# SajayR/TRIAD

Measured on AMD Instinct MI355X. Metric: tri-modal triples/sec (whole node) + loss parity, B=256 at 1/2/4/8 MI355X, higher is better.
Workload: dtype bf16

## Files before the change

triad_amd/csrc/attention.hip:

```cpp
#include "attention_tiles.h"

namespace {

constexpr int MAX_KT = 10;

struct AttnArgs {
  const bf16 *q, *k, *v, *o, *dout;
  long long q_sB, q_sN, k_sB, k_sN, v_sB, v_sN, o_sB, o_sN, do_sB, do_sN;
  bf16 *out, *dq, *dk, *dv;
  long long out_sB, out_sN, dq_sB, dq_sN, dk_sB, dk_sN, dv_sB, dv_sN;
  float* lse;
  float* delta;
  int B, H, N;
  float scale;
  const unsigned *wq, *wk;
  int nkt;
  float drop_scale;
};

template <int NT>
__device__ __forceinline__ void load_rows2(char* l0, const bf16* b0, long long s0, char* l1, const bf16* b1,
                                           long long s1, int N) {
  static_assert((NT * 32 * 8) % 256 == 0, "256 threads");
  constexpr int PER = NT * 32 * 8 / 256;
  bf16x8 r0[PER], r1[PER];
#pragma unroll
  for (int i = 0; i < PER; ++i) {
    const int e = threadIdx.x + 256 * i, r = e >> 3, c = e & 7;
    r0[i] = r < N ? *(const bf16x8*)(b0 + (long long)r * s0 + c * 8) : (bf16x8){};
    r1[i] = r < N ? *(const bf16x8*)(b1 + (long long)r * s1 + c * 8) : (bf16x8){};
  }
#pragma unroll
  for (int i = 0; i < PER; ++i) {
    const int e = threadIdx.x + 256 * i, r = e >> 3, c = e & 7;
    const int off = r * 128 + ((c ^ swz(r)) << 4);
    *(bf16x8*)(l0 + off) = r0[i];
    *(bf16x8*)(l1 + off) = r1[i];
  }
}

template <int NKT, bool DROP>
__global__ __launch_bounds__(256, 2) void attn_fwd_kernel(AttnArgs a) {
  __shared__ __attribute__((aligned(16))) char lds[2 * NKT * 32 * 128];
  char* kl = lds;
  char* vl = lds + NKT * 32 * 128;
  const int bh = blockIdx.y, b = bh / a.H, hh = bh - b * a.H;
  const int lane = threadIdx.x & 63, wave = threadIdx.x >> 6, h = lane >> 5, ql = lane & 31;
  const int qt = blockIdx.x * 4 + wave;
  const int q = qt * 32 + ql;
  const bool qok = q < a.N;
  bf16x8 qf[4];
  {
    const bf16* qp = a.q + b * a.q_sB + (long long)(qok ? q : 0) * a.q_sN + hh * HD + 8 * h;
#pragma unroll
    for (int s = 0; s < 4; ++s) qf[s] = qok ? *(const bf16x8*)(qp + 16 * s) : (bf16x8){};
  }
  load_rows2<NKT>(kl, a.k + b * a.k_sB + hh * HD, a.k_sN, vl, a.v + b * a.v_sB + hh * HD, a.v_sN, a.N);
  __syncthreads();
  if (qt * 32 >= a.N) return;
  f32x16 acc[NKT];
#pragma unroll
  for (int kt = 0; kt < NKT; ++kt) {
    acc[kt] = (f32x16){};
#pragma unroll
    for (int s = 0; s < 4; ++s) acc[kt] = mfma32(lds_b128(kl, kt * 32 + ql, 2 * s + h), qf[s], acc[kt]);
  }
  const int nlast = a.N - (NKT - 1) * 32;
  if (nlast < 32) {
#pragma unroll
    for (int v = 0; v < 16; ++v)
      if ((v & 3) + 8 * (v >> 2) + 4 * h >= nlast) acc[NKT - 1][v] = -INFINITY;
  }
  float m = -INFINITY;
#pragma unroll
  for (int kt = 0; kt < NKT; ++kt)
#pragma unroll
    for (int v = 0; v < 16; ++v) m = fmaxf(m, acc[kt][v]);
  m = fmaxf(m, __shfl_xor(m, 32));
  const float c2 = a.scale * LOG2E;
  const float mo = m * c2;
  float l = 0.f;
#pragma unroll
  for (int kt = 0; kt < NKT; ++kt)
#pragma unroll
    for (int v = 0; v < 16; ++v) {
      const float p = __builtin_amdgcn_exp2f(fmaf(acc[kt][v], c2, -mo));
      acc[kt][v] = p;
      l += p;
    }
  l += __shfl_xor(l, 32);
  if (DROP) {
#pragma unroll
    for (int kt = 0; kt < NKT; ++kt) {
      const unsigned w = qok ? a.wq[((long long)bh * a.N + q) * NKT + kt] : 0u;
#pragma unroll
      for (int v = 0; v < 16; ++v) acc[kt][v] = tile_bit(w, v, h) ? acc[kt][v] : 0.f;
    }
  }

  f32x16 o0 = {}, o1 = {};
#pragma unroll
  for (int kt = 0; kt < NKT; ++kt)
#pragma unroll
    for (int half = 0; half < 2; ++half) {
      const int c = 2 * kt + half;
      const bf16x8 pf = pack8(acc[kt], half);
      o0 = mfma32(frag_tr(vl, c, 0, lane), pf, o0);
      o1 = mfma32(frag_tr(vl, c, 32, lane), pf, o1);
    }
  if (!qok) return;
  const float inv = (DROP ? a.drop_scale : 1.f) / l;
  bf16* op = a.out + b * a.out_sB + (long long)q * a.out_sN + hh * HD;
  store_cols(op, o0, inv, h);
  store_cols(op + 32, o1, inv, h);
  if (h == 0) a.lse[(long long)bh * a.N + q] = m * a.scale + logf(l);
}

template <int NKT, bool DROP>
__global__ __launch_bounds__(256, 2) void attn_dq_kernel(AttnArgs a) {
  __shared__ __attribute__((aligned(16))) char lds[2 * NKT * 32 * 128];
  char* kl = lds;
  char* vl = lds + NKT * 32 * 128;
  const int bh = blockIdx.y, b = bh / a.H, hh = bh - b * a.H;
  const int lane = threadIdx.x & 63, wave = threadIdx.x >> 6, h = lane >> 5, ql = lane & 31;
  const int qt = blockIdx.x * 4 + wave;
  const int q = qt * 32 + ql;
  const bool qok = q < a.N;
  bf16x8 qf[4], df[4], ov[4];
  {
    const long long qq = qok ? q : 0;
    const bf16* qp = a.q + b * a.q_sB + qq * a.q_sN + hh * HD + 8 * h;
    const bf16* dp = a.dout + b * a.do_sB + qq * a.do_sN + hh * HD + 8 * h;
    const bf16* op = a.o + b * a.o_sB + qq * a.o_sN + hh * HD + 8 * h;
#pragma unroll
    for (int s = 0; s < 4; ++s) {
      qf[s] = qok ? *(const bf16x8*)(qp + 16 * s) : (bf16x8){};
      df[s] = qok ? *(const bf16x8*)(dp + 16 * s) : (bf16x8){};
      ov[s] = qok ? *(const bf16x8*)(op + 16 * s) : (bf16x8){};
    }
  }
  const float lse2 = qok ? a.lse[(long long)bh * a.N + q] * LOG2E : 0.f;
  load_rows2<NKT>(kl, a.k + b * a.k_sB + hh * HD, a.k_sN, vl, a.v + b * a.v_sB + hh * HD, a.v_sN, a.N);
  __syncthreads();
  if (qt * 32 >= a.N) return;
  float dl = 0.f;
#pragma unroll
  for (int s = 0; s < 4; ++s)
#pragma unroll
    for (int i = 0; i < 8; ++i) dl = fmaf((float)df[s][i], (float)ov[s][i], dl);
  dl += __shfl_xor(dl, 32);
  if (qok && h == 0) a.delta[(long long)bh * a.N + q] = dl;
  const float c2 = a.scale * LOG2E;
  f32x16 g0 = {}, g1 = {};
#pragma unroll
  for (int kt = 0; kt < NKT; ++kt) {
    f32x16 s = {}, dp = {};
#pragma unroll
    for (int st = 0; st < 4; ++st) {
      s = mfma32(lds_b128(kl, kt * 32 + ql, 2 * st + h), qf[st], s);
      dp = mfma32(lds_b128(vl, kt * 32 + ql, 2 * st + h), df[st], dp);
    }
    const int nv = a.N - kt * 32;
    const unsigned w = DROP && qok ? a.wq[((long long)bh * a.N + q) * NKT + kt] : 0u;
#pragma unroll
    for (int v = 0; v < 16; ++v) {
      const bool ok = qok && (v & 3) + 8 * (v >> 2) + 4 * h < nv;
      const float e = __builtin_amdgcn_exp2f(fmaf(s[v], c2, -lse2));
      const float p = ok ? e : 0.f;
      const float dpv = DROP ? (tile_bit(w, v, h) ? dp[v] * a.drop_scale : 0.f) : dp[v];
      s[v] = p * (dpv - dl);
    }
#pragma unroll
    for (int half = 0; half < 2; ++half) {
      const int c = 2 * kt + half;
      const bf16x8 sf = pack8(s, half);
      g0 = mfma32(frag_tr(kl, c, 0, lane), sf, g0);
      g1 = mfma32(frag_tr(kl, c, 32, lane), sf, g1);
    }
  }
  if (!qok) return;
  bf16* gp = a.dq + b * a.dq_sB + (long long)q * a.dq_sN + hh * HD;
  store_cols(gp, g0, a.scale, h);
  store_cols(gp + 32, g1, a.scale, h);
}

template <int NQT, bool DROP>
__global__ __launch_bounds__(256, 2) void attn_dkv_kernel(AttnArgs a) {
  __shared__ __attribute__((aligned(16))) char lds[2 * NQT * 32 * 128];
  __shared__ float stat[2][NQT * 32];
  char* ql_ = lds;
  char* dl_ = lds + NQT * 32 * 128;
  const int bh = blockIdx.y, b = bh / a.H, hh = bh - b * a.H;
  const int lane = threadIdx.x & 63, wave = threadIdx.x >> 6, h = lane >> 5, kl = lane & 31;
  const int kt = blockIdx.x * 4 + wave;
  const int key = kt * 32 + kl;
  const bool kok = key < a.N;
  bf16x8 kf[4], vf[4];
  {
    const long long kk = kok ? key : 0;
    const bf16* kp = a.k + b * a.k_sB + kk * a.k_sN + hh * HD + 8 * h;
    const bf16* vp = a.v + b * a.v_sB + kk * a.v_sN + hh * HD + 8 * h;
#pragma unroll
    for (int s = 0; s < 4; ++s) {
      kf[s] = kok ? *(const bf16x8*)(kp + 16 * s) : (bf16x8){};
      vf[s] = kok ? *(const bf16x8*)(vp + 16 * s) : (bf16x8){};
    }
  }
  load_rows2<NQT>(ql_, a.q + b * a.q_sB + hh * HD, a.q_sN, dl_, a.dout + b * a.do_sB + hh * HD, a.do_sN, a.N);
  for (int i = threadIdx.x; i < NQT * 32; i += blockDim.x) {
    const bool ok = i < a.N;
    stat[0][i] = ok ? a.lse[(long long)bh * a.N + i] * LOG2E : INFINITY;
    stat[1][i] = ok ? a.delta[(long long)bh * a.N + i] : 0.f;
  }
  __syncthreads();
  if (kt * 32 >= a.N) return;
  const float c2 = a.scale * LOG2E;
  f32x16 dv0 = {}, dv1 = {}, dk0 = {}, dk1 = {};
#pragma unroll 1
  for (int qt = 0; qt < NQT; ++qt) {
    f32x16 s = {}, dp = {};
#pragma unroll
    for (int st = 0; st < 4; ++st) {
      s = mfma32(lds_b128(ql_, qt * 32 + kl, 2 * st + h), kf[st], s);
      dp = mfma32(lds_b128(dl_, qt * 32 + kl, 2 * st + h), vf[st], dp);
    }
    const unsigned w = DROP && kok ? a.wk[((long long)bh * a.N + key) * NQT + qt] : 0u;
#pragma unroll
    for (int j = 0; j < 4; ++j) {
      const int q0 = qt * 32 + 8 * j + 4 * h;
      const f32x4 ls = *(const f32x4*)&stat[0][q0];
      const f32x4 de = *(const f32x4*)&stat[1][q0];
#pragma unroll
      for (int i = 0; i < 4; ++i) {
        const int v = 4 * j + i;
        const float e = __builtin_amdgcn_exp2f(fmaf(s[v], c2, -ls[i]));
        const float p = kok ? e : 0.f;
        if (DROP) {
          const float m = tile_bit(w, v, h) ? a.drop_scale : 0.f;
          s[v] = p * m;
          dp[v] = p * (dp[v] * m - de[i]);
        } else {
          s[v] = p;
          dp[v] = p * (dp[v] - de[i]);
        }
      }
    }
#pragma unroll
    for (int half = 0; half < 2; ++half) {
      const int c = 2 * qt + half;
      const bf16x8 pf = pack8(s, half);
      const bf16x8 sf = pack8(dp, half);
      const bf16x8 d0 = frag_tr(dl_, c, 0, lane), d1 = frag_tr(dl_, c, 32, lane);
      const bf16x8 q0 = frag_tr(ql_, c, 0, lane), q1 = frag_tr(ql_, c, 32, lane);
      dv0 = mfma32(pf, d0, dv0);
      dv1 = mfma32(pf, d1, dv1);
      dk0 = mfma32(sf, q0, dk0);
      dk1 = mfma32(sf, q1, dk1);
    }
  }
#pragma unroll
  for (int v = 0; v < 16; ++v) {
    const int kr = kt * 32 + (v & 3) + 8 * (v >> 2) + 4 * h;
    if (kr < a.N) {
      bf16* dkp = a.dk + b * a.dk_sB + (long long)kr * a.dk_sN + hh * HD + kl;
      bf16* dvp = a.dv + b * a.dv_sB + (long long)kr * a.dv_sN + hh * HD + kl;
      dkp[0] = (bf16)(dk0[v] * a.scale);
      dkp[32] = (bf16)(dk1[v] * a.scale);
      dvp[0] = (bf16)dv0[v];
      dvp[32] = (bf16)dv1[v];
    }
  }
}

#define ATTN_SWITCH(KERNEL, DR, NT, GRID, ARGS)                                                 \
  switch (NT) {                                                                                \
    case 1: hipLaunchKernelGGL((KERNEL<1, DR>), GRID, dim3(256), 0, stream, ARGS); break;       \
    case 2: hipLaunchKernelGGL((KERNEL<2, DR>), GRID, dim3(256), 0, stream, ARGS); break;       \
    case 3: hipLaunchKernelGGL((KERNEL<3, DR>), GRID, dim3(256), 0, stream, ARGS); break;       \
    case 4: hipLaunchKernelGGL((KERNEL<4, DR>), GRID, dim3(256), 0, stream, ARGS); break;       \
    case 5: hipLaunchKernelGGL((KERNEL<5, DR>), GRID, dim3(256), 0, stream, ARGS); break;       \
    case 6: hipLaunchKernelGGL((KERNEL<6, DR>), GRID, dim3(256), 0, stream, ARGS); break;       \
    case 7: hipLaunchKernelGGL((KERNEL<7, DR>), GRID, dim3(256), 0, stream, ARGS); break;       \
    case 8: hipLaunchKernelGGL((KERNEL<8, DR>), GRID, dim3(256), 0, stream, ARGS); break;       \
    case 9: hipLaunchKernelGGL((KERNEL<9, DR>), GRID, dim3(256), 0, stream, ARGS); break;       \
    default: hipLaunchKernelGGL((KERNEL<10, DR>), GRID, dim3(256), 0, stream, ARGS); break;     \
  }

__global__ __launch_bounds__(256) void attn_dropmask_kernel(int N, int nkt, unsigned seed, unsigned thr,
                                                            unsigned* __restrict__ wq, unsigned* __restrict__ wk) {
  __shared__ unsigned words[MAX_KT][33];
  const int qt = blockIdx.x;
  const long long bh = blockIdx.y;
  for (int t = threadIdx.x; t < 32 * nkt; t += 256) {
    const int r = t & 31, kt = t >> 5, q = qt * 32 + r;
    unsigned bits = 0u;
    if (q < N) {
      const unsigned long long e0 = (unsigned long long)((bh * N + q) * N + kt * 32);
      const int ncol = min(32, N - kt * 32);
      const unsigned long long p0 = e0 >> 1;
      const int off = (int)(e0 & 1);
      unsigned long long stream = 0ull;
      const int npairs = (ncol + off + 1) >> 1;
#pragma unroll
      for (int i = 0; i < 17; ++i)
        if (i < npairs) stream |= (unsigned long long)keep_pair(p0 + i, seed, thr) << (2 * i);
      bits = (unsigned)(stream >> off);
      if (ncol < 32) bits &= (1u << ncol) - 1u;
      wq[(bh * N + q) * nkt + kt] = bits;
    }
    words[kt][r] = bits;
  }
  __syncthreads();
  for (int t = threadIdx.x; t < 32 * nkt; t += 256) {
    const int j = t & 31, kt = t >> 5;
    const int key = kt * 32 + j;
    if (key < N) {
      unsigned w = 0u;
#pragma unroll
      for (int i = 0; i < 32; ++i) w |= ((words[kt][i] >> j) & 1u) << i;
      wk[(bh * N + key) * nkt + qt] = w;
    }
  }
}

bool attn_ok(int B, int H, int N, int D, float scale) {
  return B > 0 && H > 0 && N > 0 && N <= MAX_KT * 32 && D == HD && (long long)B * H <= 65535 &&
         scale > 0.f && scale < INFINITY;
}
}

extern "C" {

int triad_attn_dropmask(int B, int H, int N, float p, unsigned seed, unsigned* wq, unsigned* wk, hipStream_t stream) {
  if (B <= 0 || H <= 0 || N <= 0 || N > MAX_KT * 32 || p < 0.f || p >= 1.f || (long long)B * H > 65535)
    return TRIAD_EINVAL;
  const int nkt = (N + 31) / 32;
  hipLaunchKernelGGL(attn_dropmask_kernel, dim3(nkt, B * H), dim3(256), 0, stream, N, nkt, seed,
                     triad_drop_thr(p), wq, wk);
  TRIAD_CHECK_LAUNCH();
  return TRIAD_OK;
}

int triad_attn_fwd_dropout(const void* q, long long q_sB, long long q_sN, const void* k, long long k_sB,
                           long long k_sN, const void* v, long long v_sB, long long v_sN, int B, int H, int N, int D,
                           float scale, const unsigned* wq, float p, void* out, long long out_sB, long long out_sN,
                           float* lse, hipStream_t stream) {
  if (!attn_ok(B, H, N, D, scale) || !(p >= 0.f && p < 1.f) || !lse) return TRIAD_EINVAL;
  if (!row_ok(q, q_sB, q_sN) || !row_ok(k, k_sB, k_sN) || !row_ok(v, v_sB, v_sN) || !row_ok(out, out_sB, out_sN))
    return TRIAD_EINVAL;
  AttnArgs a = {};
  a.q = (const bf16*)q; a.q_sB = q_sB; a.q_sN = q_sN;
  a.k = (const bf16*)k; a.k_sB = k_sB; a.k_sN = k_sN;
  a.v = (const bf16*)v; a.v_sB = v_sB; a.v_sN = v_sN;
  a.out = (bf16*)out; a.out_sB = out_sB; a.out_sN = out_sN;
  a.lse = lse; a.B = B; a.H = H; a.N = N; a.scale = scale;
  const int nt = (N + 31) / 32;
  a.wq = wq; a.nkt = nt; a.drop_scale = 1.f / (1.f - p);
  const dim3 grid((nt + 3) / 4, B * H);
  if (wq) { ATTN_SWITCH(attn_fwd_kernel, true, nt, grid, a) }
  else { ATTN_SWITCH(attn_fwd_kernel, false, nt, grid, a) }
  TRIAD_CHECK_LAUNCH();
  return TRIAD_OK;
}

int triad_attn_fwd(const void* q, long long q_sB, long long q_sN, const void* k, long long k_sB, long long k_sN,
                   const void* v, long long v_sB, long long v_sN, int B, int H, int N, int D, float scale, void* out,
                   long long out_sB, long long out_sN, float* lse, hipStream_t stream) {
  return triad_attn_fwd_dropout(q, q_sB, q_sN, k, k_sB, k_sN, v, v_sB, v_sN, B, H, N, D, scale, nullptr, 0.f, out,
                                out_sB, out_sN, lse, stream);
}

int triad_attn_bwd_dropout(const void* q, long long q_sB, long long q_sN, const void* k, long long k_sB,
                           long long k_sN, const void* v, long long v_sB, long long v_sN, const void* o,
                           long long o_sB, long long o_sN, const void* dout, long long do_sB, long long do_sN,
                           const float* lse, int B, int H, int N, int D, float scale, const unsigned* wq,
                           const unsigned* wk, float p, void* dq, long long dq_sB, long long dq_sN, void* dk,
                           long long dk_sB, long long dk_sN, void* dv, long long dv_sB, long long dv_sN, float* delta,
                           hipStream_t stream) {
  if (!attn_ok(B, H, N, D, scale) || !(p >= 0.f && p < 1.f) || (!wq != !wk) || !lse || !delta) return TRIAD_EINVAL;
  if (!row_ok(q, q_sB, q_sN) || !row_ok(k, k_sB, k_sN) || !row_ok(v, v_sB, v_sN) || !row_ok(o, o_sB, o_sN) ||
      !row_ok(dout, do_sB, do_sN) || !row_ok(dq, dq_sB, dq_sN) || !row_ok(dk, dk_sB, dk_sN) ||
      !row_ok(dv, dv_sB, dv_sN))
    return TRIAD_EINVAL;
  AttnArgs a = {};
  a.q = (const bf16*)q; a.q_sB = q_sB; a.q_sN = q_sN;
  a.k = (const bf16*)k; a.k_sB = k_sB; a.k_sN = k_sN;
  a.v = (const bf16*)v; a.v_sB = v_sB; a.v_sN = v_sN;
  a.o = (const bf16*)o; a.o_sB = o_sB; a.o_sN = o_sN;
  a.dout = (const bf16*)dout; a.do_sB = do_sB; a.do_sN = do_sN;
  a.dq = (bf16*)dq; a.dq_sB = dq_sB; a.dq_sN = dq_sN;
  a.dk = (bf16*)dk; a.dk_sB = dk_sB; a.dk_sN = dk_sN;
  a.dv = (bf16*)dv; a.dv_sB = dv_sB; a.dv_sN = dv_sN;
  a.lse = (float*)lse; a.delta = delta; a.B = B; a.H = H; a.N = N; a.scale = scale;
  const int nt = (N + 31) / 32;
  a.wq = wq; a.wk = wk; a.nkt = nt; a.drop_scale = 1.f / (1.f - p);
  const dim3 grid((nt + 3) / 4, B * H);
  if (wq) {
    ATTN_SWITCH(attn_dq_kernel, true, nt, grid, a)
    ATTN_SWITCH(attn_dkv_kernel, true, nt, grid, a)
  } else {
    ATTN_SWITCH(attn_dq_kernel, false, nt, grid, a)
    ATTN_SWITCH(attn_dkv_kernel, false, nt, grid, a)
  }
  TRIAD_CHECK_LAUNCH();
  return TRIAD_OK;
}

int triad_attn_bwd(const void* q, long long q_sB, long long q_sN, const void* k, long long k_sB, long long k_sN,
                   const void* v, long long v_sB, long long v_sN, const void* o, long long o_sB, long long o_sN,
                   const void* dout, long long do_sB, long long do_sN, const float* lse, int B, int H, int N, int D,
                   float scale, void* dq, long long dq_sB, long long dq_sN, void* dk, long long dk_sB,
                   long long dk_sN, void* dv, long long dv_sB, long long dv_sN, float* delta, hipStream_t stream) {
  return triad_attn_bwd_dropout(q, q_sB, q_sN, k, k_sB, k_sN, v, v_sB, v_sN, o, o_sB, o_sN, dout, do_sB, do_sN, lse,
                                B, H, N, D, scale, nullptr, nullptr, 0.f, dq, dq_sB, dq_sN, dk, dk_sB, dk_sN, dv,
                                dv_sB, dv_sN, delta, stream);
}

}
```

Baseline: 1949.

## Use one block per head with waves looping over query/key tiles

The attention forward, dQ and dKV kernels now launch one block per (batch, head). The four waves stride over all 32-row tiles, so K/V (or Q/dO) are staged into LDS once per head instead of once per group of four tiles. Launch bounds are raised for small tile counts to allow more resident blocks. Register lifetimes are also constrained with opaque lane computation and asm barriers, and the half-wave shuffle is replaced with ds_bpermute. The trade-off is fewer blocks and more serial work per wave when sequences are long.

```diff
diff --git a/triad_amd/csrc/attention.hip b/triad_amd/csrc/attention.hip
--- a/triad_amd/csrc/attention.hip
+++ b/triad_amd/csrc/attention.hip
@@ -39,116 +39,140 @@
   }
 }
 
+__device__ __forceinline__ void row_frags(bf16x8 (&f)[4], const bf16* slice, long long sN, int row, bool ok, int h) {
+  const bf16* p = slice + (long long)row * sN + 8 * h;
+#pragma unroll
+  for (int s = 0; s < 4; ++s) f[s] = (bf16x8){};
+  if (ok) {
+#pragma unroll
+    for (int s = 0; s < 4; ++s) f[s] = *(const bf16x8*)(p + 16 * s);
+  }
+}
+
+__device__ __forceinline__ int opaque_lane() {
+  int lane;
+  asm volatile("v_mbcnt_lo_u32_b32 %0, -1, 0\n\tv_mbcnt_hi_u32_b32 %0, -1, %0" : "=v"(lane));
+  return lane;
+}
+
+__device__ __forceinline__ float other_half(float x, int lane) {
+  return __builtin_bit_cast(float, __builtin_amdgcn_ds_bpermute((lane ^ 32) << 2, __builtin_bit_cast(int, x)));
+}
+
 template <int NKT, bool DROP>
-__global__ __launch_bounds__(256, 2) void attn_fwd_kernel(AttnArgs a) {
+__device__ __forceinline__ void fwd_tile(const AttnArgs& a, const char* kl, const char* vl, int bh, int b, int hh,
+                                         int qt, const bf16x8 (&qf)[4]) {
+  f32x16 acc[NKT];
+  float m = -INFINITY, l = 0.f;
+  {
+    const int lane = opaque_lane(), h = lane >> 5, ql = lane & 31;
+#pragma unroll
+    for (int kt = 0; kt < NKT; ++kt) {
+      acc[kt] = (f32x16){};
+#pragma unroll
+      for (int s = 0; s < 4; ++s) acc[kt] = mfma32(lds_b128(kl, kt * 32 + ql, 2 * s + h), qf[s], acc[kt]);
+    }
+    const int nlast = a.N - (NKT - 1) * 32;
+    if (nlast < 32) {
+#pragma unroll
+      for (int v = 0; v < 16; ++v)
+        if ((v & 3) + 8 * (v >> 2) + 4 * h >= nlast) acc[NKT - 1][v] = -INFINITY;
+    }
+#pragma unroll
+    for (int kt = 0; kt < NKT; ++kt)
+#pragma unroll
+      for (int v = 0; v < 16; ++v) m = fmaxf(m, acc[kt][v]);
+    m = fmaxf(m, other_half(m, lane));
+    const float c2 = a.scale * LOG2E;
+    const float mo = m * c2;
+#pragma unroll
+    for (int kt = 0; kt < NKT; ++kt) {
+#pragma unroll
+      for (int v = 0; v < 16; ++v) {
+        const float p = __builtin_amdgcn_exp2f(fmaf(acc[kt][v], c2, -mo));
+        acc[kt][v] = p;
+        l += p;
+      }
+      asm volatile("" : "+v"(acc[kt]));
+    }
+    l += other_half(l, lane);
+  }
+  float inv;
+  {
+    const int lane = opaque_lane(), q = qt * 32 + (lane & 31);
+    if (q < a.N && lane < 32) a.lse[(long long)bh * a.N + q] = m * a.scale + logf(l);
+    inv = (DROP ? a.drop_scale : 1.f) / l;
+  }
+  unsigned w[NKT];
+  if (DROP) {
+    const int lane = opaque_lane(), q = qt * 32 + (lane & 31);
+#pragma unroll
+    for (int kt = 0; kt < NKT; ++kt) w[kt] = q < a.N ? a.wq[((long long)bh * a.N + q) * NKT + kt] : 0u;
+  }
+
+  f32x16 o0 = {}, o1 = {};
+  {
+    const int lane = opaque_lane(), h = lane >> 5;
+#pragma unroll
+    for (int kt = 0; kt < NKT; ++kt) {
+      if (DROP) {
+#pragma unroll
+        for (int v = 0; v < 16; ++v) acc[kt][v] = tile_bit(w[kt], v, h) ? acc[kt][v] : 0.f;
+      }
+#pragma unroll
+      for (int half = 0; half < 2; ++half) {
+        const int c = 2 * kt + half;
+        const bf16x8 pf = pack8(acc[kt], half);
+        o0 = mfma32(frag_tr(vl, c, 0, lane), pf, o0);
+        o1 = mfma32(frag_tr(vl, c, 32, lane), pf, o1);
+      }
+    }
+  }
+  const int lane = opaque_lane(), h = lane >> 5, q = qt * 32 + (lane & 31);
+  if (q >= a.N) return;
+  bf16* op = a.out + b * a.out_sB + (long long)q * a.out_sN + hh * HD;
+  store_cols(op, o0, inv, h);
+  store_cols(op + 32, o1, inv, h);
+}
+
+template <int NKT, bool DROP>
+__global__ __launch_bounds__(256, NKT <= 4 ? 4 : NKT <= 6 ? 3 : 2) void attn_fwd_kernel(AttnArgs a) {
   __shared__ __attribute__((aligned(16))) char lds[2 * NKT * 32 * 128];
   char* kl = lds;
   char* vl = lds + NKT * 32 * 128;
   const int bh = blockIdx.y, b = bh / a.H, hh = bh - b * a.H;
-  const int lane = threadIdx.x & 63, wave = threadIdx.x >> 6, h = lane >> 5, ql = lane & 31;
-  const int qt = blockIdx.x * 4 + wave;
+  const int wave = __builtin_amdgcn_readfirstlane(threadIdx.x >> 6), n = a.N;
+  const bf16* qs = a.q + b * a.q_sB + hh * HD;
+  bf16x8 qf[4];
+  {
+    const int lane = threadIdx.x & 63, q = wave * 32 + (lane & 31);
+    row_frags(qf, qs, a.q_sN, q, q < n, lane >> 5);
+  }
+  load_rows2<NKT>(kl, a.k + b * a.k_sB + hh * HD, a.k_sN, vl, a.v + b * a.v_sB + hh * HD, a.v_sN, n);
+  __syncthreads();
+  if (wave * 32 >= n) return;
+  for (int qt = wave;;) {
+    fwd_tile<NKT, DROP>(a, kl, vl, bh, b, hh, qt, qf);
+    qt += 4;
+    if (NKT <= 4 || qt * 32 >= n) break;
+    const int lane = opaque_lane(), q = qt * 32 + (lane & 31);
+    row_frags(qf, qs, a.q_sN, q, q < n, lane >> 5);
+  }
+}
+
+template <int NKT, bool DROP>
+__device__ __forceinline__ void dq_tile(const AttnArgs& a, const char* kl, const char* vl, int bh, int b, int hh,
+                                        int qt, int lane, const bf16x8 (&qf)[4], const bf16x8 (&df)[4],
+                                        const bf16x8 (&ov)[4], float lse2) {
+  const int h = lane >> 5, ql = lane & 31;
   const int q = qt * 32 + ql;
   const bool qok = q < a.N;
-  bf16x8 qf[4];
-  {
-    const bf16* qp = a.q + b * a.q_sB + (long long)(qok ? q : 0) * a.q_sN + hh * HD + 8 * h;
-#pragma unroll
-    for (int s = 0; s < 4; ++s) qf[s] = qok ? *(const bf16x8*)(qp + 16 * s) : (bf16x8){};
-  }
-  load_rows2<NKT>(kl, a.k + b * a.k_sB + hh * HD, a.k_sN, vl, a.v + b * a.v_sB + hh * HD, a.v_sN, a.N);
-  __syncthreads();
-  if (qt * 32 >= a.N) return;
-  f32x16 acc[NKT];
-#pragma unroll
-  for (int kt = 0; kt < NKT; ++kt) {
-    acc[kt] = (f32x16){};
-#pragma unroll
-    for (int s = 0; s < 4; ++s) acc[kt] = mfma32(lds_b128(kl, kt * 32 + ql, 2 * s + h), qf[s], acc[kt]);
-  }
-  const int nlast = a.N - (NKT - 1) * 32;
-  if (nlast < 32) {
-#pragma unroll
-    for (int v = 0; v < 16; ++v)
-      if ((v & 3) + 8 * (v >> 2) + 4 * h >= nlast) acc[NKT - 1][v] = -INFINITY;
-  }
-  float m = -INFINITY;
-#pragma unroll
-  for (int kt = 0; kt < NKT; ++kt)
-#pragma unroll
-    for (int v = 0; v < 16; ++v) m = fmaxf(m, acc[kt][v]);
-  m = fmaxf(m, __shfl_xor(m, 32));
-  const float c2 = a.scale * LOG2E;
-  const float mo = m * c2;
-  float l = 0.f;
-#pragma unroll
-  for (int kt = 0; kt < NKT; ++kt)
-#pragma unroll
-    for (int v = 0; v < 16; ++v) {
-      const float p = __builtin_amdgcn_exp2f(fmaf(acc[kt][v], c2, -mo));
-      acc[kt][v] = p;
-      l += p;
-    }
-  l += __shfl_xor(l, 32);
-  if (DROP) {
-#pragma unroll
-    for (int kt = 0; kt < NKT; ++kt) {
-      const unsigned w = qok ? a.wq[((long long)bh * a.N + q) * NKT + kt] : 0u;
-#pragma unroll
-      for (int v = 0; v < 16; ++v) acc[kt][v] = tile_bit(w, v, h) ? acc[kt][v] : 0.f;
-    }
-  }
-
-  f32x16 o0 = {}, o1 = {};
-#pragma unroll
-  for (int kt = 0; kt < NKT; ++kt)
-#pragma unroll
-    for (int half = 0; half < 2; ++half) {
-      const int c = 2 * kt + half;
-      const bf16x8 pf = pack8(acc[kt], half);
-      o0 = mfma32(frag_tr(vl, c, 0, lane), pf, o0);
-      o1 = mfma32(frag_tr(vl, c, 32, lane), pf, o1);
-    }
-  if (!qok) return;
-  const float inv = (DROP ? a.drop_scale : 1.f) / l;
-  bf16* op = a.out + b * a.out_sB + (long long)q * a.out_sN + hh * HD;
-  store_cols(op, o0, inv, h);
-  store_cols(op + 32, o1, inv, h);
-  if (h == 0) a.lse[(long long)bh * a.N + q] = m * a.scale + logf(l);
-}
-
-template <int NKT, bool DROP>
-__global__ __launch_bounds__(256, 2) void attn_dq_kernel(AttnArgs a) {
-  __shared__ __attribute__((aligned(16))) char lds[2 * NKT * 32 * 128];
-  char* kl = lds;
-  char* vl = lds + NKT * 32 * 128;
-  const int bh = blockIdx.y, b = bh / a.H, hh = bh - b * a.H;
-  const int lane = threadIdx.x & 63, wave = threadIdx.x >> 6, h = lane >> 5, ql = lane & 31;
-  const int qt = blockIdx.x * 4 + wave;
-  const int q = qt * 32 + ql;
-  const bool qok = q < a.N;
-  bf16x8 qf[4], df[4], ov[4];
-  {
-    const long long qq = qok ? q : 0;
-    const bf16* qp = a.q + b * a.q_sB + qq * a.q_sN + hh * HD + 8 * h;
-    const bf16* dp = a.dout + b * a.do_sB + qq * a.do_sN + hh * HD + 8 * h;
-    const bf16* op = a.o + b * a.o_sB + qq * a.o_sN + hh * HD + 8 * h;
-#pragma unroll
-    for (int s = 0; s < 4; ++s) {
-      qf[s] = qok ? *(const bf16x8*)(qp + 16 * s) : (bf16x8){};
-      df[s] = qok ? *(const bf16x8*)(dp + 16 * s) : (bf16x8){};
-      ov[s] = qok ? *(const bf16x8*)(op + 16 * s) : (bf16x8){};
-    }
-  }
-  const float lse2 = qok ? a.lse[(long long)bh * a.N + q] * LOG2E : 0.f;
-  load_rows2<NKT>(kl, a.k + b * a.k_sB + hh * HD, a.k_sN, vl, a.v + b * a.v_sB + hh * HD, a.v_sN, a.N);
-  __syncthreads();
-  if (qt * 32 >= a.N) return;
   float dl = 0.f;
 #pragma unroll
   for (int s = 0; s < 4; ++s)
 #pragma unroll
     for (int i = 0; i < 8; ++i) dl = fmaf((float)df[s][i], (float)ov[s][i], dl);
-  dl += __shfl_xor(dl, 32);
+  dl += other_half(dl, lane);
   if (qok && h == 0) a.delta[(long long)bh * a.N + q] = dl;
   const float c2 = a.scale * LOG2E;
   f32x16 g0 = {}, g1 = {};
@@ -184,36 +208,46 @@
   store_cols(gp + 32, g1, a.scale, h);
 }
 
+struct DqRows {
+  bf16x8 qf[4], df[4], ov[4];
+  float lse2;
+};
+__device__ __forceinline__ void dq_rows(DqRows& r, const AttnArgs& a, int bh, int b, int hh, int n, int qt, int lane) {
+  const int h = lane >> 5, q = qt * 32 + (lane & 31);
+  const bool qok = q < n;
+  row_frags(r.qf, a.q + b * a.q_sB + hh * HD, a.q_sN, q, qok, h);
+  row_frags(r.df, a.dout + b * a.do_sB + hh * HD, a.do_sN, q, qok, h);
+  row_frags(r.ov, a.o + b * a.o_sB + hh * HD, a.o_sN, q, qok, h);
+  r.lse2 = qok ? a.lse[(long long)bh * a.N + q] * LOG2E : 0.f;
+}
+
+template <int NKT, bool DROP>
+__global__ __launch_bounds__(256, NKT == 1 ? 4 : NKT <= 6 ? 3 : 2) void attn_dq_kernel(AttnArgs a) {
+  __shared__ __attribute__((aligned(16))) char lds[2 * NKT * 32 * 128];
+  char* kl = lds;
+  char* vl = lds + NKT * 32 * 128;
+  const int bh = blockIdx.y, b = bh / a.H, hh = bh - b * a.H;
+  const int wave = __builtin_amdgcn_readfirstlane(threadIdx.x >> 6), n = a.N;
+  DqRows r;
+  dq_rows(r, a, bh, b, hh, n, wave, threadIdx.x & 63);
+  load_rows2<NKT>(kl, a.k + b * a.k_sB + hh * HD, a.k_sN, vl, a.v + b * a.v_sB + hh * HD, a.v_sN, n);
+  __syncthreads();
+  if (wave * 32 >= n) return;
+  for (int qt = wave;;) {
+    dq_tile<NKT, DROP>(a, kl, vl, bh, b, hh, qt, opaque_lane(), r.qf, r.df, r.ov, r.lse2);
+    qt += 4;
+    if (NKT <= 4 || qt * 32 >= n) break;
+    dq_rows(r, a, bh, b, hh, n, qt, opaque_lane());
+  }
+}
+
 template <int NQT, bool DROP>
-__global__ __launch_bounds__(256, 2) void attn_dkv_kernel(AttnArgs a) {
-  __shared__ __attribute__((aligned(16))) char lds[2 * NQT * 32 * 128];
-  __shared__ float stat[2][NQT * 32];
-  char* ql_ = lds;
-  char* dl_ = lds + NQT * 32 * 128;
-  const int bh = blockIdx.y, b = bh / a.H, hh = bh - b * a.H;
-  const int lane = threadIdx.x & 63, wave = threadIdx.x >> 6, h = lane >> 5, kl = lane & 31;
-  const int kt = blockIdx.x * 4 + wave;
+__device__ __forceinline__ void dkv_tile(const AttnArgs& a, const char* ql_, const char* dl_, const float (&stat)[2][NQT * 32],
+                                         int bh, int b, int hh, int kt, int lane, const bf16x8 (&kf)[4],
+                                         const bf16x8 (&vf)[4]) {
+  const int h = lane >> 5, kl = lane & 31;
   const int key = kt * 32 + kl;
   const bool kok = key < a.N;
-  bf16x8 kf[4], vf[4];
-  {
-    const long long kk = kok ? key : 0;
-    const bf16* kp = a.k + b * a.k_sB + kk * a.k_sN + hh * HD + 8 * h;
-    const bf16* vp = a.v + b * a.v_sB + kk * a.v_sN + hh * HD + 8 * h;
-#pragma unroll
-    for (int s = 0; s < 4; ++s) {
-      kf[s] = kok ? *(const bf16x8*)(kp + 16 * s) : (bf16x8){};
-      vf[s] = kok ? *(const bf16x8*)(vp + 16 * s) : (bf16x8){};
-    }
-  }
-  load_rows2<NQT>(ql_, a.q + b * a.q_sB + hh * HD, a.q_sN, dl_, a.dout + b * a.do_sB + hh * HD, a.do_sN, a.N);
-  for (int i = threadIdx.x; i < NQT * 32; i += blockDim.x) {
-    const bool ok = i < a.N;
-    stat[0][i] = ok ? a.lse[(long long)bh * a.N + i] * LOG2E : INFINITY;
-    stat[1][i] = ok ? a.delta[(long long)bh * a.N + i] : 0.f;
-  }
-  __syncthreads();
-  if (kt * 32 >= a.N) return;
   const float c2 = a.scale * LOG2E;
   f32x16 dv0 = {}, dv1 = {}, dk0 = {}, dk1 = {};
 #pragma unroll 1
@@ -269,6 +303,40 @@
       dvp[0] = (bf16)dv0[v];
       dvp[32] = (bf16)dv1[v];
     }
+  }
+}
+
+template <int NQT, bool DROP>
+__global__ __launch_bounds__(256, NQT == 1 ? 4 : 2) void attn_dkv_kernel(AttnArgs a) {
+  __shared__ __attribute__((aligned(16))) char lds[2 * NQT * 32 * 128];
+  __shared__ __attribute__((aligned(16))) float stat[2][NQT * 32];
+  char* ql_ = lds;
+  char* dl_ = lds + NQT * 32 * 128;
+  const int bh = blockIdx.y, b = bh / a.H, hh = bh - b * a.H;
+  const int wave = __builtin_amdgcn_readfirstlane(threadIdx.x >> 6), n = a.N;
+  const bf16* ks = a.k + b * a.k_sB + hh * HD;
+  const bf16* vs = a.v + b * a.v_sB + hh * HD;
+  bf16x8 kf[4], vf[4];
+  {
+    const int lane = threadIdx.x & 63, key = wave * 32 + (lane & 31);
+    row_frags(kf, ks, a.k_sN, key, key < n, lane >> 5);
+    row_frags(vf, vs, a.v_sN, key, key < n, lane >> 5);
+  }
+  load_rows2<NQT>(ql_, a.q + b * a.q_sB + hh * HD, a.q_sN, dl_, a.dout + b * a.do_sB + hh * HD, a.do_sN, n);
+  for (int i = threadIdx.x; i < NQT * 32; i += blockDim.x) {
+    const bool ok = i < n;
+    stat[0][i] = ok ? a.lse[(long long)bh * a.N + i] * LOG2E : INFINITY;
+    stat[1][i] = ok ? a.delta[(long long)bh * a.N + i] : 0.f;
+  }
+  __syncthreads();
+  if (wave * 32 >= n) return;
+  for (int kt = wave;;) {
+    dkv_tile<NQT, DROP>(a, ql_, dl_, stat, bh, b, hh, kt, opaque_lane(), kf, vf);
+    kt += 4;
+    if (NQT <= 4 || kt * 32 >= n) break;
+    const int lane = opaque_lane(), key = kt * 32 + (lane & 31);
+    row_frags(kf, ks, a.k_sN, key, key < n, lane >> 5);
+    row_frags(vf, vs, a.v_sN, key, key < n, lane >> 5);
   }
 }
 
@@ -356,7 +424,7 @@
   a.lse = lse; a.B = B; a.H = H; a.N = N; a.scale = scale;
   const int nt = (N + 31) / 32;
   a.wq = wq; a.nkt = nt; a.drop_scale = 1.f / (1.f - p);
-  const dim3 grid((nt + 3) / 4, B * H);
+  const dim3 grid(1, B * H);
   if (wq) { ATTN_SWITCH(attn_fwd_kernel, true, nt, grid, a) }
   else { ATTN_SWITCH(attn_fwd_kernel, false, nt, grid, a) }
   TRIAD_CHECK_LAUNCH();
@@ -394,7 +462,7 @@
   a.lse = (float*)lse; a.delta = delta; a.B = B; a.H = H; a.N = N; a.scale = scale;
   const int nt = (N + 31) / 32;
   a.wq = wq; a.wk = wk; a.nkt = nt; a.drop_scale = 1.f / (1.f - p);
-  const dim3 grid((nt + 3) / 4, B * H);
+  const dim3 grid(1, B * H);
   if (wq) {
     ATTN_SWITCH(attn_dq_kernel, true, nt, grid, a)
     ATTN_SWITCH(attn_dkv_kernel, true, nt, grid, a)
```

New measurement: 1947. No clear change (-0.1%).
